# rland93/rrtplanner

Measured on AMD Instinct MI355X. Metric: RRT* nodes-expanded/s on 1024x1024 Perlin grid; achieved HBM GB/s, higher is better.
Workload: dtype int16x2 coordinates / u32 squared distances / f64 costs; 1 GPU; BASELINE.json configs[1]: RRT* 1024x1024 n=50000 r_rewire=64; queries_per_gpu=1, total_queries=1, n=50000, unfinished_queries=0, cus_per_query=65, pipelined=True, team_fallbacks=0, collective_library=librccl.so.1

## Files before the change

### include/rrt_hip.h

```cpp
#ifndef RRT_HIP_H
#define RRT_HIP_H

#include <stdint.h>

#ifdef __cplusplus
extern "C" {
#endif

#define RRT_OK 0
#define RRT_NEED_UNITBALL 1
#define RRT_E_ARG (-1)
#define RRT_E_GOAL_UNREACHABLE (-2)
#define RRT_E_HIP (-3)
#define RRT_E_NOGRID (-4)
#define RRT_E_UNSUPPORTED (-5)
#define RRT_E_COMM (-6)

#define RRT_ALG_STANDARD 0
#define RRT_ALG_STAR 1
#define RRT_ALG_INFORMED 2
#define RRT_ALG_DUBINS 3
#define RRT_ALG_DUBINS_STAR 4

#define RRT_FLAG_LOGS 1u
#define RRT_FLAG_SERIAL 2u
#define RRT_FLAG_NOTEAM 4u
#define RRT_FLAG_TEAM_FAULT 8u
#define RRT_FLAG_NOPIPE 16u
#define RRT_FLAG_REWIRE 32u
#define RRT_FLAG_DUBINS 64u
#define RRT_FLAG_NOPIPE1 32768u
#define RRT_FLAG_TEAM_MAX(g) ((uint32_t)(g) << 8)

typedef struct rrt_ctx rrt_ctx;
typedef struct rrt_batch rrt_batch;

typedef struct rrt_query {
    int32_t alg;
    int32_t n;
    int32_t xs[2];
    int32_t xg[2];
    int64_t r2_rewire;
    int64_t goal_d2;
    const int32_t *samples;
    double C[4];
    const int32_t *headings;
    double rho;
    int32_t nh;
    int32_t hs, hg;
    int32_t pad_;
    const uint32_t *samples_packed;
} rrt_query;

typedef struct rrt_result {
    int32_t *pts;
    double *vcost;
    int32_t *parent;
    int32_t *nearest_log;
    uint8_t *accept_log;
    double *cbest_log;
    int32_t *j_log;
    int32_t status;
    int32_t j;
// ... 76 lines not shown
```

### rrtplanner_amd/_ffi.py

```python
import ctypes as C
import weakref
import os

import numpy as np

_HERE = os.path.dirname(os.path.abspath(__file__))
LIB_PATH = os.environ.get("RRT_HIP_LIB", os.path.join(_HERE, "librrt_hip.so"))

RRT_OK = 0
RRT_NEED_UNITBALL = 1
RRT_E_ARG = -1
RRT_E_GOAL_UNREACHABLE = -2
RRT_E_HIP = -3
RRT_E_NOGRID = -4
RRT_E_UNSUPPORTED = -5
RRT_E_COMM = -6

ALG_STANDARD, ALG_STAR, ALG_INFORMED = 0, 1, 2
ALG_DUBINS, ALG_DUBINS_STAR = 3, 4
FLAG_LOGS = 1
FLAG_SERIAL = 2
FLAG_NOTEAM = 4
FLAG_TEAM_FAULT = 8
FLAG_NOPIPE = 16
FLAG_REWIRE = 32
FLAG_DUBINS = 64
FLAG_NOPIPE1 = 32768


def kernel_flags(logs=False, serial=False, team=None, team_fault=False, pipe=True, rewire=False, dubins=False, pipe1=True):
    f = (FLAG_LOGS if logs else 0) | (FLAG_SERIAL if serial else 0) | (FLAG_TEAM_FAULT if team_fault else 0) | (0 if pipe else FLAG_NOPIPE)
    f |= FLAG_REWIRE if rewire else 0
    f |= FLAG_DUBINS if dubins else 0
    f |= 0 if pipe1 else FLAG_NOPIPE1
    if team == 1:
        f |= FLAG_NOTEAM
    elif team is not None:
        if team not in (2, 3, 4, 8, 16, 32, 64):
            raise ValueError("team must be None, 1, 2, 3, 4, 8, 16, 32 or 64")
        f |= int(team) << 8
    return f

SYMBOLS = (
    "rrt_ctx_create", "rrt_ctx_destroy", "rrt_last_error_string", "rrt_set_grid", "rrt_noise_grids", "rrt_select_frame",
    "rrt_grid_generation", "rrt_ctx_sync",
    "rrt_comm_use_library", "rrt_comm_unique_id", "rrt_comm_init", "rrt_comm_destroy", "rrt_comm_allreduce_f64", "rrt_gather", "rrt_gather_fetch",
    "rrt_batch_create", "rrt_batch_destroy", "rrt_batch_set_query", "rrt_batch_set_unitball",
    "rrt_batch_rearm", "rrt_batch_launch", "rrt_batch_sync", "rrt_batch_team", "rrt_batch_team_info", "rrt_batch_pipelined", "rrt_batch_kernel_name", "rrt_batch_elapsed_ms",
    "rrt_batch_get_result", "rrt_batch_result_block", "rrt_batch_debug_cycles",
    "rrt_plan", "rrt_plan_resume", "rrt_plan_batch",
    "rrt_tree_create", "rrt_tree_destroy", "rrt_tree_reset", "rrt_tree_append", "rrt_tree_query",
    "rrt_prim_collisionfree", "rrt_prim_nearest_within", "rrt_prim_sqrt_u32", "rrt_prim_sqrt_u24", "rrt_prim_sqrt_f64",
)


class RRTError(RuntimeError):
    def __init__(self, code, msg):
        super().__init__(f"librrt_hip error {code}: {msg}")
        self.code = code


class Query(C.Structure):
    _fields_ = [
        ("alg", C.c_int32), ("n", C.c_int32),
        ("xs", C.c_int32 * 2), ("xg", C.c_int32 * 2),
        ("r2_rewire", C.c_int64), ("goal_d2", C.c_int64),
        ("samples", C.c_void_p),
# ... 199 lines not shown
                                              cells.ctypes.data, amps.ctypes.data, grads.ctypes.data, out.ctypes.data))
        self.shape = (W, H)
        return out

    def select_frame(self, k):
        _check(self._h, lib().rrt_select_frame(self._h, int(k)))

    def grid_generation(self):
        g = C.c_uint64(0)
        _check(self._h, lib().rrt_grid_generation(self._h, C.byref(g)))
        return g.value

    def sync(self):
        _check(self._h, lib().rrt_ctx_sync(self._h))

    def comm_init(self, rank, world, unique_id: bytes):
        if len(unique_id) != COMM_ID_BYTES:
            raise ValueError(f"unique id must have {COMM_ID_BYTES} bytes")
        buf = (C.c_uint8 * COMM_ID_BYTES).from_buffer_copy(unique_id)
        _check(self._h, lib().rrt_comm_init(self._h, int(rank), int(world), C.cast(buf, C.c_void_p)))
        self.rank, self.world = int(rank), int(world)

    def comm_destroy(self):
        _check(self._h, lib().rrt_comm_destroy(self._h))

    def allreduce(self, values, op="sum"):
        v = np.ascontiguousarray(values, dtype=np.float64).copy()
        _check(self._h, lib().rrt_comm_allreduce_f64(self._h, v.ctypes.data, v.size, {"sum": 0, "max": 1, "min": 2}[op]))
        return v

    def barrier(self):
        self.allreduce([0.0])

    def plan(self, query, n, logs=False, serial=False, team=None, team_fault=False, pipe=True, rewire=False, pipe1=True):
        res = ResultArrays(n, logs, headings=query.alg >= ALG_DUBINS)
        flags = kernel_flags(logs, serial, team, team_fault, pipe, rewire, pipe1=pipe1)
        rc = lib().rrt_plan(self._h, C.byref(query), flags, C.byref(res.c))
        _check(self._h, rc, ok=(RRT_OK, RRT_NEED_UNITBALL, RRT_E_GOAL_UNREACHABLE))
        return rc, res

    def plan_resume(self, unitball, res):
        ub = np.ascontiguousarray(unitball, dtype=np.float64)
        rc = lib().rrt_plan_resume(self._h, ub.ctypes.data, ub.shape[0], C.byref(res.c))
        _check(self._h, rc, ok=(RRT_OK, RRT_NEED_UNITBALL, RRT_E_GOAL_UNREACHABLE))
        return rc

    def plan_batch(self, queries, ns):
        Q = len(queries)
        qarr = (Query * Q)(*queries)
        res = [ResultArrays(int(n)) for n in ns]
        rarr = (Result * Q)(*[r.c for r in res])
        rc = lib().rrt_plan_batch(self._h, Q, qarr, rarr)
        _check(self._h, rc, ok=(RRT_OK, RRT_NEED_UNITBALL, RRT_E_GOAL_UNREACHABLE))
        for r, c in zip(res, rarr):
            r.c = c
        return rc, res

    def prim_collisionfree(self, ab):
        ab = np.ascontiguousarray(ab, dtype=np.int32).reshape(-1, 4)
        m = ab.shape[0]
        free = np.zeros(m, dtype=np.uint8)
        cells = np.zeros(m, dtype=np.int32)
        _check(self._h, lib().rrt_prim_collisionfree(self._h, ab.ctypes.data, m, free.ctypes.data, cells.ctypes.data))
        return free.astype(bool), cells

    def prim_nearest_within(self, pts, xq, r2):
        pts = np.ascontiguousarray(pts, dtype=np.int32).reshape(-1, 2)
        xq = np.ascontiguousarray(xq, dtype=np.int32).reshape(-1, 2)
        m = xq.shape[0]
# ... 33 lines not shown
        self._idx = np.zeros(self.capacity, dtype=np.int32)
        self._los = np.zeros(self.capacity + 1, dtype=np.uint8)

    def close(self):
        if self._h:
            lib().rrt_tree_destroy(self._h)
            self._h = C.c_void_p()

    def __del__(self):
        try:
            self.close()
        except Exception:
            pass

    def reset(self):
        _check(self.ctx.handle, lib().rrt_tree_reset(self._h))

    def append(self, x, y) -> int:
        j = C.c_int32(-1)
        _check(self.ctx.handle, lib().rrt_tree_append(self._h, int(x), int(y), C.byref(j)))
        return j.value

    def query(self, x, y, r2):
        nn, cnt = C.c_int32(-1), C.c_int32(0)
        _check(self.ctx.handle, lib().rrt_tree_query(self._h, int(x), int(y), int(r2), C.byref(nn), C.byref(cnt), self._idx.ctypes.data,
                                                     self._los.ctypes.data, self.capacity))
        m = cnt.value
        return nn.value, self._idx[:m].copy(), bool(self._los[0]), self._los[1:1 + m].astype(bool)


class Batch:

    def __init__(self, ctx: Context, Q: int, n_cap: int, logs: bool = False, serial: bool = False, team=None, team_fault: bool = False,
                 pipe: bool = True, rewire: bool = False, dubins: bool = False, pipe1: bool = True):
        self.ctx, self.Q, self.n_cap, self.logs, self.dubins = ctx, int(Q), int(n_cap), logs, dubins
        self._h = C.c_void_p()
        flags = kernel_flags(logs, serial, team, team_fault, pipe, rewire, dubins, pipe1)
        _check(ctx.handle, lib().rrt_batch_create(ctx.handle, self.Q, self.n_cap, flags, C.byref(self._h)))
        if not hasattr(ctx, "_batches"):
            ctx._batches = weakref.WeakSet()
        ctx._batches.add(self)
        self._n = [0] * self.Q

    def close(self):
        if self._h:
            lib().rrt_batch_destroy(self._h)
            self._h = C.c_void_p()

    def __del__(self):
        try:
            self.close()
        except Exception:
            pass

    def set_query(self, q, query):
        _check(self.ctx.handle, lib().rrt_batch_set_query(self._h, int(q), C.byref(query)))
        self._n[q] = query.n

    def set_unitball(self, q, unitball, ub_offset):
        ub = np.ascontiguousarray(unitball, dtype=np.float64)
        _check(self.ctx.handle, lib().rrt_batch_set_unitball(self._h, int(q), ub.ctypes.data, ub.shape[0], int(ub_offset)))

    def rearm(self):
        _check(self.ctx.handle, lib().rrt_batch_rearm(self._h))

    def launch(self):
        _check(self.ctx.handle, lib().rrt_batch_launch(self._h))

    def sync(self):
        _check(self.ctx.handle, lib().rrt_batch_sync(self._h))
# ... 57 lines not shown
```

### rrtplanner_amd/csrc/kernels_tu.hip

```cpp
#include <hip/hip_runtime.h>

#if RRT_TU == 1
#define RRT_BLOCK_DECL_ONLY
#define RRT_SERIAL_DECL_ONLY
#include "rrt_pipe.h"

#elif RRT_TU == 2
#include "rrt_dubins_block.h"
namespace rrtdev {
template __global__ void rrt_expand_kernel<false, true>(BatchView);
}

#elif RRT_TU == 3
#include "rrt_kernels.h"
namespace rrtdev {
template __global__ void rrt_expand_kernel<false, false>(BatchView);
template __global__ void rrt_expand_kernel<true, false>(BatchView);
}

#else
#define RRT_SERIAL_DECL_ONLY
#include "rrt_block.h"
namespace rrtdev {
#define K(G, BSM, PIPE, INF) template __global__ void rrt_expand_block_kernel<G, BSM, PIPE, INF>(BatchView);
#if RRT_TU == 10
K(64, 1, true, false)
#elif RRT_TU == 11
K(64, 1, true, true)
#elif RRT_TU == 12
K(32, 2, true, false) K(32, 2, true, true)
#elif RRT_TU == 13
K(16, 4, true, false) K(16, 4, true, true)
#elif RRT_TU == 14
K(8, 8, true, false) K(8, 8, true, true)
#elif RRT_TU == 15
K(4, 16, true, false) K(4, 16, true, true)
#elif RRT_TU == 16
K(3, 16, true, false) K(3, 16, true, true)
#elif RRT_TU == 17
K(2, 16, true, false) K(2, 16, true, true) K(2, 32, true, false)
#elif RRT_TU == 18
K(64, 1, false, false) K(64, 1, false, true) K(32, 2, false, false) K(32, 2, false, true)
#elif RRT_TU == 19
K(16, 4, false, false) K(16, 4, false, true) K(8, 8, false, false) K(8, 8, false, true)
#elif RRT_TU == 20
K(4, 16, false, false) K(4, 16, false, true) K(2, 16, false, false) K(2, 16, false, true)
#elif RRT_TU == 21
K(1, 16, false, false) K(1, 16, false, true)
#else
#error "RRT_TU: unknown translation unit"
#endif
#undef K
}
#endif
```

### rrtplanner_amd/csrc/rrt_block.h

```cpp
#pragma once

#include "rrt_kernels.h"

namespace rrtdev {

constexpr int BS = 16;

constexpr int TEAM_MAX = 64;
#ifndef RRT_PIPE_LAG
#define RRT_PIPE_LAG 2
#endif
#ifndef RRT_PIPE_LAG_SMALL
#define RRT_PIPE_LAG_SMALL 1
#endif
#ifndef RRT_PIPE_LAG_INF
#define RRT_PIPE_LAG_INF 2
#endif
#ifndef RRT_NPMAX
#define RRT_NPMAX 2
#endif
constexpr int NPMAX = RRT_NPMAX;
#ifndef RRT_PL_MAX
#define RRT_PL_MAX 12
#endif
// ... 759 lines not shown
#ifdef RRT_STAMPS
    if (lane == 0 && !PIPE) {
        D->wcyc[wave] = wcyc_acc;
        D->wcyc[16 + wave] = wcyc_los;
    }
    if (PIPE && t == 0 && g <= 1)
#pragma unroll
        for (int k = 0; k < 16; ++k) D->wcyc[16 * g + k] = dbg[k];
#endif
}

template <int G, int BSM, bool PIPE, bool INF>
__global__ __launch_bounds__(TPB) void rrt_expand_block_kernel(BatchView bv)
#ifdef RRT_BLOCK_DECL_ONLY
    ;
#else
{
    __shared__ BlockLds<G, BSM, PIPE, INF> L;
    if constexpr (PIPE) {
#if defined(RRT_ONLY_ROLE) && RRT_ONLY_ROLE == 1
        rrt_block_body<G, BSM, PIPE, INF, ROLE_COMMIT>(bv, L);
#elif defined(RRT_ONLY_ROLE) && RRT_ONLY_ROLE == 2
        rrt_block_body<G, BSM, PIPE, INF, ROLE_WORK>(bv, L);
#else
        if ((int)blockIdx.x < bv.team_qpad) rrt_block_body<G, BSM, PIPE, INF, ROLE_COMMIT>(bv, L);
        else rrt_block_body<G, BSM, PIPE, INF, ROLE_WORK>(bv, L);
#endif
    } else {
        rrt_block_body<G, BSM, PIPE, INF, ROLE_ALL>(bv, L);
    }
}
#endif

}
```

### rrtplanner_amd/csrc/rrt_block_nearset.inc

```

    constexpr bool GQ = PIPE && ROLE == ROLE_WORK && BSM < 16;
    constexpr uint32_t OQCAP = (uint32_t)(SB * BREC_WORDS * 8 / 16 / (BSM < 16 ? BSM : 1));
    constexpr bool GLIST = false;
    constexpr bool LDSLIST = BSM >= 16 || GLIST;
    constexpr uint32_t LCAP = BSM >= 16 ? (uint32_t)BLOCK_LIST_CAP : (uint32_t)(SB * BREC_WORDS * 8 / 16 / NWAVE);
    const uint32_t clist_cap = (uint32_t)(bv.spill_stride / (2 * NWAVE * (G + (PIPE ? 1 : 0))));
    u32x4 *const clist_base = reinterpret_cast<u32x4 *>(spill) + (size_t)(g * NWAVE) * (size_t)clist_cap;
    u32x4 *const clist = clist_base + (size_t)wave * (size_t)clist_cap;
    RRT_LDS u32x4 *const clist_l =
        GLIST ? (RRT_LDS u32x4 *)&brec[PIPE ? 1 : 0][0] + (size_t)wave * LCAP
              : (RRT_LDS u32x4 *)(smem + (size_t)lds_chunks * CHUNK * sizeof(uint32_t) + (size_t)MAX_CELLS * sizeof(uint32_t)) + (size_t)wave * LCAP;
    auto lget = [&](uint32_t p) -> u32x4 {
        if (LDSLIST && p < LCAP) return clist_l[p];
        return clist[p];
    };
    auto lput = [&](uint32_t p, u32x4 e) {
        if (LDSLIST && p < LCAP) clist_l[p] = e;
        else clist[p] = e;
    };
    auto lput_y = [&](uint32_t p, uint32_t y) {
        if (LDSLIST && p < LCAP) clist_l[p].y = y;
        else clist[p].y = y;
    };
    RRT_LDS u32x4 *const clist_l0 = clist_l - (size_t)wave * LCAP;
// ... 46 lines not shown
        uint32_t ld2 = NONE, lidx = NONE;
        nlist = 0;
        float T = boundf;
        uint32_t Thi = hi_of((double)boundf);
        auto eval_record = [&](const u32x4 rc, bool &dirty) {
            const uint32_t d2 = dist2(rc.x, X);
            const bool hit = d2 < r2h && (!check_j0 || rc.y < (uint32_t)j0);
            hits += hit ? 1u : 0u;
            if (hit && (d2 < ld2 || (d2 == ld2 && rc.y < lidx))) {
                ld2 = d2;
                lidx = rc.y;
                lxy = rc.x;
                lvlo = rc.z;
                lvhi = rc.w;
            }
            if (!star) return;
            const bool park = hit && rc.w <= boundhi;
            const unsigned long long pm = __ballot(park);
            if (pm == 0) return;
            if (park) {
                const uint32_t pos = nlist + (uint32_t)__builtin_popcountll(pm & ((1ull << lane) - 1ull));
                if (pos < clist_cap) lput(pos, u32x4{rc.y, rc.x, rc.z, rc.w});
            }
            nlist += (uint32_t)__builtin_popcountll(pm);
            const bool pre = park && rc.w <= Thi;
            if (__ballot(pre) == 0) return;
            const double V = __longlong_as_double((long long)(((unsigned long long)rc.w << 32) | rc.z));
            const bool maybe = pre && ((float)V + __builtin_amdgcn_sqrtf((float)d2) < T);
            if (__ballot(maybe) == 0) return;
            if (maybe) {
                const double cn = V + sqrt_u24(d2);
                const bool in = cn < bound && !key_lt(cn, rc.y, lbc, lbi);
                if (in) {
                    if (key_lt(cn, rc.y, tt.c1, tt.i1)) {
                        fx2 = fx1;
                        fx1 = rc.x;
                    } else if (key_lt(cn, rc.y, tt.c2, tt.i2)) {
                        fx2 = rc.x;
                    }
                    tt.fold(cn, rc.y);
                }
                const float cu = in ? screen_of(cn) : FINF;
                const float lo = __builtin_fminf(m1, cu), hi = __builtin_fmaxf(m1, cu);
                m1 = lo;
                m2 = __builtin_fminf(m2, hi);
            }
            dirty = true;
        };
        auto tighten = [&]() {
            const float w1 = wave_min_f32_nonneg(m1);
            const float w2 = wave_min_f32_nonneg(m1 == w1 ? m2 : m1);
            T = w2 < boundf ? w2 : boundf;
            Thi = hi_of((double)T);
        };
        for (int cbase = 0; cbase < ncr; cbase += 64) {
            uint32_t tcnt = 0, toff = 0;
            if (cbase + lane < ncr) {
                const int ci = cbase + lane, ccx = cx0 + ci / ny, ccy = cy0 + ci % ny, cell = ccx * ncy + ccy;
#ifndef RRT_NO_CELL_CULL
                const int xl = ccx << cshift, xh = xl + (1 << cshift) - 1, yl = ccy << cshift, yh = yl + (1 << cshift) - 1;
                const int ddx = x < xl ? xl - x : (x > xh ? x - xh : 0), ddy = y < yl ? yl - y : (y > yh ? y - yh : 0);
                tcnt = (uint32_t)(ddx * ddx + ddy * ddy) < r2h ? cellcnt[cell] : 0u;
#else
                tcnt = cellcnt[cell];
#endif
                toff = (uint32_t)cell * (uint32_t)ccap;
            }
            uint32_t incl = tcnt;
            incl += (uint32_t)__builtin_amdgcn_update_dpp(0, (int)incl, 0x111, 0xf, 0xf, false);
            incl += (uint32_t)__builtin_amdgcn_update_dpp(0, (int)incl, 0x112, 0xf, 0xf, false);
            incl += (uint32_t)__builtin_amdgcn_update_dpp(0, (int)incl, 0x114, 0xf, 0xf, false);
            incl += (uint32_t)__builtin_amdgcn_update_dpp(0, (int)incl, 0x118, 0xf, 0xf, false);
// ... 262 lines not shown
```

### rrtplanner_amd/csrc/rrt_engine.hip

```cpp
#include <hip/hip_runtime.h>
#include <rccl/rccl.h>
#include <dlfcn.h>

#include <chrono>
#include <cmath>
#include <cstdarg>
#include <cstdio>
#include <cstdlib>
#include <cstring>
#include <mutex>
#include <string>
#include <tuple>
#include <vector>

#define RRT_BLOCK_DECL_ONLY
#define RRT_SERIAL_DECL_ONLY
#include "rrt_hip.h"
#include "rrt_kernels.h"
#include "rrt_block.h"
#include "rrt_kernel_decls.h"
#include "rrt_prims.h"

using namespace rrtdev;

static thread_local std::string g_last_error;

constexpr int RRT_GRID_FAST = 2048;
constexpr int RRT_GRID_MAX = 32767;

struct PinnedDescs {
    QDesc *p = nullptr;
    size_t n = 0;
    hipError_t alloc(size_t count) {
        release();
        hipError_t e = hipHostMalloc(reinterpret_cast<void **>(&p), count * sizeof(QDesc), hipHostMallocDefault);
        if (e != hipSuccess) {
            p = nullptr;
            return e;
        }
        n = count;
        for (size_t k = 0; k < n; ++k) p[k] = QDesc{};
        return hipSuccess;
    }
    void release() {
        if (p) (void)hipHostFree(p);
        p = nullptr;
        n = 0;
    }
    QDesc *data() { return p; }
    QDesc *begin() { return p; }
    QDesc *end() { return p + n; }
    QDesc &operator[](size_t k) { return p[k]; }
};

struct rrt_ctx {
    int device = 0;
    hipStream_t stream = nullptr;
    uint8_t *og = nullptr;
    uint8_t *og_buf = nullptr;
    size_t og_buf_bytes = 0;
    int32_t nframes = 1;
    int32_t W = 0, H = 0;
    std::string err;
    rrt_batch *single = nullptr;
    uint32_t single_flags = 0;
    int max_lds = 0;
    int num_cu = 0;
    uint64_t grid_gen = 0;
    ncclComm_t comm = nullptr;
    int32_t comm_rank = 0, comm_world = 1;
    unsigned char *gather_buf = nullptr;
    size_t gather_bytes = 0;
    const rrt_batch *gather_owner = nullptr;
    double *d_red = nullptr;
};

struct rrt_batch {
    rrt_ctx *ctx = nullptr;
    int32_t Q = 0, n_cap = 0, node_stride = 0, bitmap_words = 0, lds_chunks = 1, spill_stride = 0;
    int32_t gridW = 0, gridH = 0;
    uint32_t flags = 0;
    bool use_block = false;
    bool dub_block = false;
    int32_t blk_lds_chunks = 1;
    int32_t blk_lds_chunks16 = 1;
    int32_t team = 1;
    bool pipe_team = false;
    bool pipe = false;
    int32_t last_team = 0;
    bool last_inf = false;
    bool last_pipe1 = false;
    bool last_wide = false;
    int32_t team_fallbacks = 0;
    int32_t team_qpad = 0;
    int32_t team_want = TEAM_MAX;
    int32_t claimed_cus = 0;
    int32_t shrunk = 0;
    unsigned char *d_team = nullptr;
    QDesc *d_desc = nullptr;
    PinnedDescs h_desc;
    size_t serial_lds_static = 0;
    uint32_t *d_samples = nullptr, *d_nodes = nullptr, *d_bitmap = nullptr;
    double *d_vcost = nullptr, *d_unitball = nullptr, *d_cbest_log = nullptr;
    int32_t *d_parent = nullptr, *d_nearest_log = nullptr, *d_j_log = nullptr;
    uint8_t *d_accept_log = nullptr;
    uint2 *d_spill = nullptr;
    int32_t *d_kids = nullptr;
    uint32_t *d_frontier = nullptr;
    int32_t *d_vsoln = nullptr;
    uint8_t *d_heading = nullptr;
    uint8_t *d_shead = nullptr;
    double *d_dubpath = nullptr;
    std::vector<uint8_t> stage8;
    uint4 *d_cellrec = nullptr;
    uint32_t *d_cellcnt = nullptr;
    int64_t rec_stride = 0;
    unsigned char *d_slab = nullptr;
    size_t slab_bytes = 0;
    hipEvent_t ev0 = nullptr, ev1 = nullptr;
    bool timed = false;
    float ms_before = 0.f;
    bool one_cu_once = false;
    std::vector<uint32_t> stage;
};

static const void *block_kernel_of(int team, bool pipe, bool inf);
static size_t block_kernel_static_lds(int team);

static hipError_t raise_dynamic_lds(int device, const void *kern, int bytes) {
    static std::mutex mu;
    static std::vector<std::tuple<int, const void *, int>> have;
    std::lock_guard<std::mutex> lock(mu);
    for (auto &t : have)
        if (std::get<0>(t) == device && std::get<1>(t) == kern) {
            if (std::get<2>(t) >= bytes) return hipSuccess;
            const hipError_t e = hipFuncSetAttribute(kern, hipFuncAttributeMaxDynamicSharedMemorySize, bytes);
            if (e == hipSuccess) std::get<2>(t) = bytes;
            return e;
        }
    const hipError_t e = hipFuncSetAttribute(kern, hipFuncAttributeMaxDynamicSharedMemorySize, bytes);
    if (e == hipSuccess) have.emplace_back(device, kern, bytes);
    return e;
}

static int fail(rrt_ctx *ctx, int code, const char *fmt, ...) {
    char buf[512];
    va_list ap;
    va_start(ap, fmt);
    vsnprintf(buf, sizeof buf, fmt, ap);
    va_end(ap);
    g_last_error = buf;
    if (ctx) ctx->err = buf;
// ... 34 lines not shown
        return e;
    }
};

extern "C" const char *rrt_last_error_string(rrt_ctx *ctx) { return ctx ? ctx->err.c_str() : g_last_error.c_str(); }

extern "C" int rrt_ctx_create(int32_t device_id, rrt_ctx **out) {
    if (!out) return fail(nullptr, RRT_E_ARG, "rrt_ctx_create: out is NULL");
    int ndev = 0;
    HIPCHK(nullptr, hipGetDeviceCount(&ndev));
    if (device_id < 0 || device_id >= ndev)
        return fail(nullptr, RRT_E_ARG, "rrt_ctx_create: device %d of %d", device_id, ndev);
    HIPCHK(nullptr, hipSetDevice(device_id));
    rrt_ctx *c = new rrt_ctx();
    c->device = device_id;
    hipError_t e = hipStreamCreateWithFlags(&c->stream, hipStreamNonBlocking);
    if (e == hipSuccess) e = hipDeviceGetAttribute(&c->max_lds, hipDeviceAttributeMaxSharedMemoryPerBlock, device_id);
    if (e == hipSuccess) e = hipDeviceGetAttribute(&c->num_cu, hipDeviceAttributeMultiprocessorCount, device_id);
    if (e != hipSuccess) {
        if (c->stream) (void)hipStreamDestroy(c->stream);
        delete c;
        return fail(nullptr, RRT_E_HIP, "rrt_ctx_create: %s", hipGetErrorString(e));
    }
    *out = c;
    return RRT_OK;
}

extern "C" int rrt_ctx_destroy(rrt_ctx *ctx) {
    if (!ctx) return RRT_OK;
    (void)hipSetDevice(ctx->device);
    if (ctx->single) rrt_batch_destroy(ctx->single);
    (void)rrt_comm_destroy(ctx);
    if (ctx->og_buf) (void)hipFree(ctx->og_buf);
    if (ctx->stream) (void)hipStreamDestroy(ctx->stream);
    delete ctx;
    return RRT_OK;
}

extern "C" int rrt_set_grid(rrt_ctx *ctx, const uint8_t *og_nonzero, int32_t W, int32_t H) {
    if (!ctx || !og_nonzero || W < 1 || H < 1) return fail(ctx, RRT_E_ARG, "rrt_set_grid: bad argument");
    if (W > RRT_GRID_MAX || H > RRT_GRID_MAX)
        return fail(ctx, RRT_E_UNSUPPORTED, "rrt_set_grid: %dx%d exceeds %d cells per axis (16-bit packed coordinates)", W, H, RRT_GRID_MAX);
    HIPCHK(ctx, hipSetDevice(ctx->device));
    HIPCHK(ctx, hipStreamSynchronize(ctx->stream));
    if (ctx->og_buf && ctx->og_buf_bytes != (size_t)W * H) {
        ctx->grid_gen += 1;
        ctx->og = nullptr;
        HIPCHK(ctx, hipFree(ctx->og_buf));
        ctx->og_buf = nullptr;
    }
    if (!ctx->og_buf) {
        HIPCHK(ctx, hipMalloc(&ctx->og_buf, (size_t)W * H));
        ctx->og_buf_bytes = (size_t)W * H;
    }
    ctx->og = ctx->og_buf;
    ctx->nframes = 1;
    ctx->grid_gen += 1;
    HIPCHK(ctx, hipMemcpyAsync(ctx->og, og_nonzero, (size_t)W * H, hipMemcpyHostToDevice, ctx->stream));
    HIPCHK(ctx, hipStreamSynchronize(ctx->stream));
    ctx->W = W;
    ctx->H = H;
    return RRT_OK;
}

namespace {
__device__ __forceinline__ double fade5(double t) { return t * t * t * (t * (t * 6.0 - 15.0) + 10.0); }
// ... 161 lines not shown

namespace {
std::mutex g_cu_mutex;
std::vector<int> g_cu_claimed;
int cu_claim(int device, int num_cu, int want_cus, int min_cus) {
    std::lock_guard<std::mutex> lock(g_cu_mutex);
    if ((int)g_cu_claimed.size() <= device) g_cu_claimed.resize((size_t)device + 1, 0);
    const int free_cus = num_cu - g_cu_claimed[(size_t)device];
    if (want_cus <= free_cus || want_cus <= min_cus) {
        g_cu_claimed[(size_t)device] += want_cus;
        return -1;
    }
    return free_cus < 0 ? 0 : free_cus;
}
void cu_release(int device, int cus) {
    if (cus <= 0) return;
    std::lock_guard<std::mutex> lock(g_cu_mutex);
    if ((int)g_cu_claimed.size() > device) g_cu_claimed[(size_t)device] -= cus;
}
}

extern "C" int rrt_batch_destroy(rrt_batch *b) {
    if (!b) return RRT_OK;
    (void)hipSetDevice(b->ctx->device);
    (void)hipStreamSynchronize(b->ctx->stream);
    void *ptrs[] = {b->d_desc,  b->d_samples,   b->d_slab,        b->d_bitmap, b->d_unitball,  b->d_cellrec,
                    b->d_spill, b->d_cbest_log, b->d_nearest_log, b->d_j_log,  b->d_accept_log, b->d_cellcnt,
                    b->d_team,  b->d_kids,      b->d_frontier,    b->d_vsoln,  b->d_heading,   b->d_shead,
                    b->d_dubpath};
    for (void *p : ptrs)
        if (p) (void)hipFree(p);
    if (b->ev0) (void)hipEventDestroy(b->ev0);
    if (b->ev1) (void)hipEventDestroy(b->ev1);
    cu_release(b->ctx->device, b->claimed_cus);
    b->claimed_cus = 0;
    if (b->ctx->single == b) b->ctx->single = nullptr;
    if (b->ctx->gather_owner == b) b->ctx->gather_owner = nullptr;
    b->h_desc.release();
    delete b;
    return RRT_OK;
}

struct TeamShape {
    int team = 1, qpad = 0;
    bool pipe = false;
    int cus() const { return team > 1 ? qpad * (team + (pipe ? 1 : 0)) : 0; }
};
static TeamShape pick_team(int Q, int want, bool allow_pipe, int cus);
static bool two_cus_run_the_pipeline(const rrt_batch *b);
static TeamShape pick_team(int Q, int want, bool allow_pipe, int cus) {
    TeamShape t;
    t.qpad = (Q + 7) & ~7;
    auto stride_of = [&](int g) {
        const int step = g <= 16 ? 8 : (g == 32 ? 4 : 2);
        int stride = ((Q + step - 1) / step) * step;
        if (g == 32 && stride % 8 == 0) stride += 4;
        if (g == 64 && stride % 4 == 0) stride += 2;
        return stride;
    };
    for (int g : {2, 4, 8, 16, 32, 64})
        if (g <= want && stride_of(g) * g <= cus) {
            t.team = g;
            t.qpad = stride_of(g);
        }
    int pipe_g = 0;
    if (allow_pipe)
// ... 288 lines not shown
    if constexpr (!INF) {
        if (pipe && wide && team == 2) return rrt_expand_block_kernel<2, 32, true, false>;
    }
    if (pipe) {
        switch (team) {
            case 64: return rrt_expand_block_kernel<64, 1, true, INF>;
            case 32: return rrt_expand_block_kernel<32, 2, true, INF>;
            case 16: return rrt_expand_block_kernel<16, 4, true, INF>;
            case 8: return rrt_expand_block_kernel<8, 8, true, INF>;
            case 4: return rrt_expand_block_kernel<4, 16, true, INF>;
            case 3: return rrt_expand_block_kernel<3, 16, true, INF>;
            default: return rrt_expand_block_kernel<2, 16, true, INF>;
        }
    }
    switch (team) {
        case 64: return rrt_expand_block_kernel<64, 1, false, INF>;
        case 32: return rrt_expand_block_kernel<32, 2, false, INF>;
        case 16: return rrt_expand_block_kernel<16, 4, false, INF>;
        case 8: return rrt_expand_block_kernel<8, 8, false, INF>;
        case 4: return rrt_expand_block_kernel<4, 16, false, INF>;
        case 2: return rrt_expand_block_kernel<2, 16, false, INF>;
        default: return rrt_expand_block_kernel<1, 16, false, INF>;
    }
}

static block_kernel_fn block_kernel_fn_of(int team, bool pipe, bool inf, bool wide = false) {
    return inf ? block_kernel_fn_inf<true>(team, pipe, wide) : block_kernel_fn_inf<false>(team, pipe, wide);
}

static const void *block_kernel_of(int team, bool pipe, bool inf, bool wide = false) {
    return reinterpret_cast<const void *>(block_kernel_fn_of(team, pipe, inf, wide));
}

static size_t block_kernel_static_lds(int team) {
    hipFuncAttributes a{};
    size_t worst = 0;
    for (int g : {1, 2, 3, 4, 8, 16, 32, 64})
        for (bool pipe : {false, true})
            for (bool inf : {false, true}) {
                if (g > team || (pipe && g < 2)) continue;
                if (!pipe && g == 3) continue;
                for (bool wide : {false, true}) {
                    if (wide && !(pipe && g == 2)) continue;
                    if (hipFuncGetAttributes(&a, block_kernel_of(g, pipe, inf, wide)) != hipSuccess) return 16384;
                    worst = a.sharedSizeBytes > worst ? a.sharedSizeBytes : worst;
                }
            }
    return (worst + 255) & ~(size_t)255;
}

static size_t expand_lds_bytes(int lds_chunks) {
    return (size_t)lds_chunks * CHUNK * sizeof(uint32_t);
}

static bool two_cus_run_the_pipeline(const rrt_batch *b) {
    return b->use_block && b->team == 2 && !b->pipe_team && b->team_want >= TEAM_MAX && !(b->flags & (RRT_FLAG_NOPIPE | RRT_FLAG_NOPIPE1));
}

extern "C" int rrt_batch_launch(rrt_batch *b) {
    if (!b) return fail(nullptr, RRT_E_ARG, "rrt_batch_launch: NULL");
    rrt_ctx *ctx = b->ctx;
    if (!ctx->og) return fail(ctx, RRT_E_NOGRID, "rrt_batch_launch: no grid");
    if (b->gridW != ctx->W || b->gridH != ctx->H) return fail(ctx, RRT_E_ARG, "rrt_batch_launch: grid changed shape");
    HIPCHK(ctx, hipSetDevice(ctx->device));
    if (!b->one_cu_once) b->ms_before = 0.f;
    BatchView v = make_view(b);
// ... 27 lines not shown
            if (ts.team != team) b->shrunk += 1;
            team = ts.team;
            pipe_shape = ts.pipe;
            v.team_qpad = ts.qpad;
            b->claimed_cus = team > 1 ? ts.cus() : 0;
        }
        if (team <= 1) {
            team = 1;
            b->claimed_cus = b->Q < ctx->num_cu ? b->Q : ctx->num_cu;
            (void)cu_claim(ctx->device, ctx->num_cu, b->claimed_cus, b->claimed_cus);
        }
        const bool lists = team <= 4;
        v.lds_chunks = lists ? b->blk_lds_chunks16 : b->blk_lds_chunks;
        const size_t blk_lds_bytes = (size_t)MAX_CELLS * sizeof(uint32_t) + (lists ? BLOCK_LIST_LDS_BYTES : 0) + (size_t)v.lds_chunks * CHUNK * sizeof(uint32_t);
        bool pipe = team > 1 && pipe_shape;
#ifdef RRT_STAMPS
        if (const char *e = getenv("RRT_PIPE")) pipe = pipe && atoi(e) != 0;
#endif
        b->pipe = pipe;
        bool inf = false;
        for (const QDesc &d : b->h_desc)
            if (d.status == ST_RUNNING && d.alg == 2) inf = true;
#ifndef RRT_NO_WIDE
        bool wide = pipe && !inf && team == 2;
        for (const QDesc &d : b->h_desc)
            if (d.status == ST_RUNNING && d.alg != RRT_ALG_STANDARD && d.r2_rewire < 257u) wide = false;
#else
        const bool wide = false;
#endif
        b->last_wide = wide;
        b->last_team = team;
        b->last_inf = inf;
        b->last_pipe1 = false;
        if (team == 1 && !inf && !continuation && !(b->flags & RRT_FLAG_NOPIPE1)) {
            b->last_pipe1 = true;
            hipLaunchKernelGGL(rrt_init_kernel<0>, ig, dim3(256), 0, ctx->stream, v);
            HIPCHK(ctx, hipEventRecord(b->ev0, ctx->stream));
            hipLaunchKernelGGL(rrt_pipe_kernel, dim3((unsigned)b->Q), dim3(TPB), 0, ctx->stream, v);
            HIPCHK(ctx, hipEventRecord(b->ev1, ctx->stream));
            HIPCHK(ctx, hipGetLastError());
            b->timed = true;
            return RRT_OK;
        }
        HIPCHK(ctx, raise_dynamic_lds(ctx->device, block_kernel_of(team, pipe, inf, wide), (int)blk_lds_bytes));
        hipLaunchKernelGGL(rrt_init_kernel<0>, ig, dim3(256), 0, ctx->stream, v);
        if (team > 1) HIPCHK(ctx, hipMemsetAsync(b->d_team, 0, (size_t)b->Q * TEAM_BYTES, ctx->stream));
        HIPCHK(ctx, hipEventRecord(b->ev0, ctx->stream));
        const dim3 tg(team > 1 ? (unsigned)(v.team_qpad * (team + (pipe ? 1 : 0))) : (unsigned)b->Q);
        hipLaunchKernelGGL(block_kernel_fn_of(team, pipe, inf, wide), tg, dim3(TPB), blk_lds_bytes, ctx->stream, v);
        HIPCHK(ctx, hipEventRecord(b->ev1, ctx->stream));
        HIPCHK(ctx, hipGetLastError());
        b->timed = true;
        return RRT_OK;
    }
    cu_release(ctx->device, b->claimed_cus);
    b->claimed_cus = b->Q < ctx->num_cu ? b->Q : ctx->num_cu;
    (void)cu_claim(ctx->device, ctx->num_cu, b->claimed_cus, b->claimed_cus);
    if (b->dub_block) {
        hipLaunchKernelGGL(rrt_init_kernel<0>, ig, dim3(256), 0, ctx->stream, v);
        HIPCHK(ctx, hipEventRecord(b->ev0, ctx->stream));
        hipLaunchKernelGGL(rrt_dubins_block_kernel, dim3((unsigned)b->Q), dim3(TPB), 0, ctx->stream, v);
        HIPCHK(ctx, hipEventRecord(b->ev1, ctx->stream));
        HIPCHK(ctx, hipGetLastError());
        b->timed = true;
        return RRT_OK;
    }
    const size_t lds = expand_lds_bytes(b->lds_chunks);
    typedef void (*serial_kernel_fn)(BatchView);
    const serial_kernel_fn kern = (b->flags & RRT_FLAG_DUBINS)  ? static_cast<serial_kernel_fn>(rrt_expand_kernel<false, true>)
                                  : (b->flags & RRT_FLAG_REWIRE) ? static_cast<serial_kernel_fn>(rrt_expand_kernel<true, false>)
                                                                 : static_cast<serial_kernel_fn>(rrt_expand_kernel<false, false>);
    if (b->serial_lds_static == 0) {
        hipFuncAttributes fa{};
        HIPCHK(ctx, hipFuncGetAttributes(&fa, reinterpret_cast<const void *>(kern)));
        b->serial_lds_static = fa.sharedSizeBytes + 1;
    }
    const size_t lds_static = b->serial_lds_static - 1;
    if ((int)(lds + lds_static) > ctx->max_lds) return fail(ctx, RRT_E_HIP, "LDS request %zu exceeds %d", lds + lds_static, ctx->max_lds);
    HIPCHK(ctx, raise_dynamic_lds(ctx->device, reinterpret_cast<const void *>(kern), (int)lds));
    hipLaunchKernelGGL(rrt_init_kernel<0>, ig, dim3(256), 0, ctx->stream, v);
    HIPCHK(ctx, hipEventRecord(b->ev0, ctx->stream));
    hipLaunchKernelGGL(kern, dim3((unsigned)b->Q), dim3(TPB), lds, ctx->stream, v);
// ... 64 lines not shown
    }
    return RRT_OK;
}

extern "C" int rrt_batch_team(rrt_batch *b, int32_t *cus_per_query, int32_t *fallbacks) {
    if (!b || !cus_per_query) return fail(nullptr, RRT_E_ARG, "rrt_batch_team: NULL");
    *cus_per_query = b->use_block ? b->team : 1;
    if (fallbacks) *fallbacks = b->team_fallbacks;
    return RRT_OK;
}

extern "C" int rrt_batch_team_info(rrt_batch *b, int32_t out[4]) {
    if (!b || !out) return fail(nullptr, RRT_E_ARG, "rrt_batch_team_info: NULL");
    out[0] = b->use_block ? b->team : 1;
    out[1] = b->use_block ? (b->last_team > 0 ? b->last_team : b->team) : 1;
    out[2] = b->team_fallbacks;
    out[3] = b->shrunk;
    return RRT_OK;
}

extern "C" int rrt_batch_pipelined(rrt_batch *b, int32_t *pipelined) {
    if (!b || !pipelined) return fail(nullptr, RRT_E_ARG, "rrt_batch_pipelined: NULL");
    *pipelined = (b->use_block && b->team > 1 && b->pipe) ? 1 : 0;
    return RRT_OK;
}

extern "C" int rrt_batch_kernel_name(rrt_batch *b, char *buf, int32_t len) {
    if (!b || !buf || len < 1) return fail(nullptr, RRT_E_ARG, "rrt_batch_kernel_name: bad argument");
    char tmp[160];
    if (b->use_block) {
        const int team = b->last_team > 0 ? b->last_team : b->team;
        const int bsm = b->last_wide ? 32 : (team <= 4 ? 16 : 64 / team);
        if (b->last_pipe1) snprintf(tmp, sizeof tmp, "rrt_pipe_kernel");
        else snprintf(tmp, sizeof tmp, "rrt_expand_block_kernel<%d, %d, %s, %s>", team, bsm, (team > 1 && b->pipe) ? "true" : "false", b->last_inf ? "true" : "false");
    } else if (b->dub_block) {
        snprintf(tmp, sizeof tmp, "rrt_dubins_block_kernel");
    } else {
        snprintf(tmp, sizeof tmp, "rrt_expand_kernel<%s, %s>", (b->flags & RRT_FLAG_REWIRE) ? "true" : "false", (b->flags & RRT_FLAG_DUBINS) ? "true" : "false");
    }
    snprintf(buf, (size_t)len, "%s", tmp);
    return RRT_OK;
}

extern "C" int rrt_batch_elapsed_ms(rrt_batch *b, float *ms) {
    if (!b || !ms) return fail(nullptr, RRT_E_ARG, "rrt_batch_elapsed_ms: NULL");
    if (!b->timed) return fail(b->ctx, RRT_E_ARG, "rrt_batch_elapsed_ms: nothing launched");
    HIPCHK(b->ctx, hipEventElapsedTime(ms, b->ev0, b->ev1));
    *ms += b->ms_before;
    return RRT_OK;
}

extern "C" int rrt_batch_get_result(rrt_batch *b, int32_t q, rrt_result *out) {
    if (!b || !out) return fail(nullptr, RRT_E_ARG, "rrt_batch_get_result: NULL");
    rrt_ctx *ctx = b->ctx;
    if (q < 0 || q >= b->Q) return fail(ctx, RRT_E_ARG, "rrt_batch_get_result: q=%d of %d", q, b->Q);
    HIPCHK(ctx, hipSetDevice(ctx->device));
    const QDesc &d = b->h_desc[(size_t)q];
    if (d.status == ST_RUNNING || d.status == ST_IDLE)
        return fail(ctx, RRT_E_ARG, "rrt_batch_get_result: query %d has not run (launch + sync first)", q);
    out->status = d.status;
    out->j = d.j;
    out->vgoal = d.vgoal;
    out->found = d.found;
    out->i_switch = d.i_switch;
    out->rows = d.found ? d.n + 1 : d.n;
    out->sum_j = (int64_t)d.sum_j;
// ... 564 lines not shown
```

Baseline: 6.000 million nodes/s.

## Split pipelined team kernel into separate commit and work kernels on two streams

For pipelined teams of 8 or more, the single fused block kernel is replaced by a commit kernel (512 threads, one block per query) launched on a second stream and a work kernel on the main stream, joined by events. Each role can then be compiled with its own launch bounds and register budget instead of sharing one body. The near-set update is also rewritten from nested branches into branchless selects. The two kernels rely on co-residency for their inter-block handshake, which creates deadlock or scheduling risk if they are not both resident.

```diff
diff --git a/include/rrt_hip.h b/include/rrt_hip.h
--- a/include/rrt_hip.h
+++ b/include/rrt_hip.h
@@ -29,6 +29,7 @@
 #define RRT_FLAG_NOPIPE 16u
 #define RRT_FLAG_REWIRE 32u
 #define RRT_FLAG_DUBINS 64u
+#define RRT_FLAG_ONEBODY 128u
 #define RRT_FLAG_NOPIPE1 32768u
 #define RRT_FLAG_TEAM_MAX(g) ((uint32_t)(g) << 8)
 
diff --git a/rrtplanner_amd/_ffi.py b/rrtplanner_amd/_ffi.py
--- a/rrtplanner_amd/_ffi.py
+++ b/rrtplanner_amd/_ffi.py
@@ -25,14 +25,16 @@
 FLAG_NOPIPE = 16
 FLAG_REWIRE = 32
 FLAG_DUBINS = 64
+FLAG_ONEBODY = 128
 FLAG_NOPIPE1 = 32768
 
 
-def kernel_flags(logs=False, serial=False, team=None, team_fault=False, pipe=True, rewire=False, dubins=False, pipe1=True):
+def kernel_flags(logs=False, serial=False, team=None, team_fault=False, pipe=True, rewire=False, dubins=False, pipe1=True, onebody=False):
     f = (FLAG_LOGS if logs else 0) | (FLAG_SERIAL if serial else 0) | (FLAG_TEAM_FAULT if team_fault else 0) | (0 if pipe else FLAG_NOPIPE)
     f |= FLAG_REWIRE if rewire else 0
     f |= FLAG_DUBINS if dubins else 0
     f |= 0 if pipe1 else FLAG_NOPIPE1
+    f |= FLAG_ONEBODY if onebody else 0
     if team == 1:
         f |= FLAG_NOTEAM
     elif team is not None:
@@ -298,9 +300,9 @@
     def barrier(self):
         self.allreduce([0.0])
 
-    def plan(self, query, n, logs=False, serial=False, team=None, team_fault=False, pipe=True, rewire=False, pipe1=True):
+    def plan(self, query, n, logs=False, serial=False, team=None, team_fault=False, pipe=True, rewire=False, pipe1=True, onebody=False):
         res = ResultArrays(n, logs, headings=query.alg >= ALG_DUBINS)
-        flags = kernel_flags(logs, serial, team, team_fault, pipe, rewire, pipe1=pipe1)
+        flags = kernel_flags(logs, serial, team, team_fault, pipe, rewire, pipe1=pipe1, onebody=onebody)
         rc = lib().rrt_plan(self._h, C.byref(query), flags, C.byref(res.c))
         _check(self._h, rc, ok=(RRT_OK, RRT_NEED_UNITBALL, RRT_E_GOAL_UNREACHABLE))
         return rc, res
@@ -400,10 +402,10 @@
 class Batch:
 
     def __init__(self, ctx: Context, Q: int, n_cap: int, logs: bool = False, serial: bool = False, team=None, team_fault: bool = False,
-                 pipe: bool = True, rewire: bool = False, dubins: bool = False, pipe1: bool = True):
+                 pipe: bool = True, rewire: bool = False, dubins: bool = False, pipe1: bool = True, onebody: bool = False):
         self.ctx, self.Q, self.n_cap, self.logs, self.dubins = ctx, int(Q), int(n_cap), logs, dubins
         self._h = C.c_void_p()
-        flags = kernel_flags(logs, serial, team, team_fault, pipe, rewire, dubins, pipe1)
+        flags = kernel_flags(logs, serial, team, team_fault, pipe, rewire, dubins, pipe1, onebody)
         _check(ctx.handle, lib().rrt_batch_create(ctx.handle, self.Q, self.n_cap, flags, C.byref(self._h)))
         if not hasattr(ctx, "_batches"):
             ctx._batches = weakref.WeakSet()
diff --git a/rrtplanner_amd/csrc/kernels_tu.hip b/rrtplanner_amd/csrc/kernels_tu.hip
--- a/rrtplanner_amd/csrc/kernels_tu.hip
+++ b/rrtplanner_amd/csrc/kernels_tu.hip
@@ -23,6 +23,9 @@
 #include "rrt_block.h"
 namespace rrtdev {
 #define K(G, BSM, PIPE, INF) template __global__ void rrt_expand_block_kernel<G, BSM, PIPE, INF>(BatchView);
+#define S(G, BSM, INF)                                                        \
+    template __global__ void rrt_block_commit_kernel<G, BSM, INF>(BatchView); \
+    template __global__ void rrt_block_work_kernel<G, BSM, INF>(BatchView);
 #if RRT_TU == 10
 K(64, 1, true, false)
 #elif RRT_TU == 11
@@ -47,9 +50,16 @@
 K(4, 16, false, false) K(4, 16, false, true) K(2, 16, false, false) K(2, 16, false, true)
 #elif RRT_TU == 21
 K(1, 16, false, false) K(1, 16, false, true)
+#elif RRT_TU == 22
+S(64, 1, false)
+#elif RRT_TU == 23
+S(32, 2, false)
+#elif RRT_TU == 24
+S(16, 4, false) S(8, 8, false)
 #else
 #error "RRT_TU: unknown translation unit"
 #endif
 #undef K
+#undef S
 }
 #endif
diff --git a/rrtplanner_amd/csrc/rrt_block.h b/rrtplanner_amd/csrc/rrt_block.h
--- a/rrtplanner_amd/csrc/rrt_block.h
+++ b/rrtplanner_amd/csrc/rrt_block.h
@@ -815,4 +815,26 @@
 }
 #endif
 
-}
+template <int G, int BSM, bool INF>
+__global__ __launch_bounds__(512) void rrt_block_commit_kernel(BatchView bv)
+#ifdef RRT_BLOCK_DECL_ONLY
+    ;
+#else
+{
+    __shared__ BlockLds<G, BSM, true, INF> L;
+    rrt_block_body<G, BSM, true, INF, ROLE_COMMIT, 8>(bv, L);
+}
+#endif
+
+template <int G, int BSM, bool INF>
+__global__ __launch_bounds__(TPB) void rrt_block_work_kernel(BatchView bv)
+#ifdef RRT_BLOCK_DECL_ONLY
+    ;
+#else
+{
+    __shared__ BlockLds<G, BSM, true, INF> L;
+    rrt_block_body<G, BSM, true, INF, ROLE_WORK>(bv, L);
+}
+#endif
+
+}
diff --git a/rrtplanner_amd/csrc/rrt_block_nearset.inc b/rrtplanner_amd/csrc/rrt_block_nearset.inc
--- a/rrtplanner_amd/csrc/rrt_block_nearset.inc
+++ b/rrtplanner_amd/csrc/rrt_block_nearset.inc
@@ -102,12 +102,10 @@
                 const double cn = V + sqrt_u24(d2);
                 const bool in = cn < bound && !key_lt(cn, rc.y, lbc, lbi);
                 if (in) {
-                    if (key_lt(cn, rc.y, tt.c1, tt.i1)) {
-                        fx2 = fx1;
-                        fx1 = rc.x;
-                    } else if (key_lt(cn, rc.y, tt.c2, tt.i2)) {
-                        fx2 = rc.x;
-                    }
+                    const bool b1 = key_lt(cn, rc.y, tt.c1, tt.i1);
+                    const bool b2 = key_lt(cn, rc.y, tt.c2, tt.i2);
+                    fx2 = b1 ? fx1 : (b2 ? rc.x : fx2);
+                    fx1 = b1 ? rc.x : fx1;
                     tt.fold(cn, rc.y);
                 }
                 const float cu = in ? screen_of(cn) : FINF;
diff --git a/rrtplanner_amd/csrc/rrt_engine.hip b/rrtplanner_amd/csrc/rrt_engine.hip
--- a/rrtplanner_amd/csrc/rrt_engine.hip
+++ b/rrtplanner_amd/csrc/rrt_engine.hip
@@ -56,6 +56,7 @@
 struct rrt_ctx {
     int device = 0;
     hipStream_t stream = nullptr;
+    hipStream_t stream2 = nullptr;
     uint8_t *og = nullptr;
     uint8_t *og_buf = nullptr;
     size_t og_buf_bytes = 0;
@@ -91,6 +92,7 @@
     bool last_inf = false;
     bool last_pipe1 = false;
     bool last_wide = false;
+    bool last_split = false;
     int32_t team_fallbacks = 0;
     int32_t team_qpad = 0;
     int32_t team_want = TEAM_MAX;
@@ -118,6 +120,7 @@
     unsigned char *d_slab = nullptr;
     size_t slab_bytes = 0;
     hipEvent_t ev0 = nullptr, ev1 = nullptr;
+    hipEvent_t ev_fork = nullptr, ev_join = nullptr;
     bool timed = false;
     float ms_before = 0.f;
     bool one_cu_once = false;
@@ -218,6 +221,7 @@
     if (ctx->single) rrt_batch_destroy(ctx->single);
     (void)rrt_comm_destroy(ctx);
     if (ctx->og_buf) (void)hipFree(ctx->og_buf);
+    if (ctx->stream2) (void)hipStreamDestroy(ctx->stream2);
     if (ctx->stream) (void)hipStreamDestroy(ctx->stream);
     delete ctx;
     return RRT_OK;
@@ -445,6 +449,8 @@
         if (p) (void)hipFree(p);
     if (b->ev0) (void)hipEventDestroy(b->ev0);
     if (b->ev1) (void)hipEventDestroy(b->ev1);
+    if (b->ev_fork) (void)hipEventDestroy(b->ev_fork);
+    if (b->ev_join) (void)hipEventDestroy(b->ev_join);
     cu_release(b->ctx->device, b->claimed_cus);
     b->claimed_cus = 0;
     if (b->ctx->single == b) b->ctx->single = nullptr;
@@ -799,6 +805,19 @@
     return reinterpret_cast<const void *>(block_kernel_fn_of(team, pipe, inf, wide));
 }
 
+static bool split_team(int team, bool pipe, bool inf, bool wide, uint32_t flags) {
+    return pipe && !inf && !wide && team >= 8 && !(flags & RRT_FLAG_ONEBODY);
+}
+
+static void split_kernels_of(int team, block_kernel_fn &commit, block_kernel_fn &work) {
+    switch (team) {
+        case 64: commit = rrt_block_commit_kernel<64, 1, false>, work = rrt_block_work_kernel<64, 1, false>; break;
+        case 32: commit = rrt_block_commit_kernel<32, 2, false>, work = rrt_block_work_kernel<32, 2, false>; break;
+        case 16: commit = rrt_block_commit_kernel<16, 4, false>, work = rrt_block_work_kernel<16, 4, false>; break;
+        default: commit = rrt_block_commit_kernel<8, 8, false>, work = rrt_block_work_kernel<8, 8, false>; break;
+    }
+}
+
 static size_t block_kernel_static_lds(int team) {
     hipFuncAttributes a{};
     size_t worst = 0;
@@ -892,6 +911,7 @@
         b->last_team = team;
         b->last_inf = inf;
         b->last_pipe1 = false;
+        b->last_split = false;
         if (team == 1 && !inf && !continuation && !(b->flags & RRT_FLAG_NOPIPE1)) {
             b->last_pipe1 = true;
             hipLaunchKernelGGL(rrt_init_kernel<0>, ig, dim3(256), 0, ctx->stream, v);
@@ -902,12 +922,35 @@
             b->timed = true;
             return RRT_OK;
         }
-        HIPCHK(ctx, raise_dynamic_lds(ctx->device, block_kernel_of(team, pipe, inf, wide), (int)blk_lds_bytes));
+        const bool split = split_team(team, pipe, inf, wide, b->flags);
+        block_kernel_fn kcommit = nullptr, kwork = nullptr;
+        if (split) {
+            split_kernels_of(team, kcommit, kwork);
+            if (!ctx->stream2) HIPCHK(ctx, hipStreamCreateWithFlags(&ctx->stream2, hipStreamNonBlocking));
+            if (!b->ev_fork) HIPCHK(ctx, hipEventCreateWithFlags(&b->ev_fork, hipEventDisableTiming));
+            if (!b->ev_join) HIPCHK(ctx, hipEventCreateWithFlags(&b->ev_join, hipEventDisableTiming));
+            HIPCHK(ctx, raise_dynamic_lds(ctx->device, reinterpret_cast<const void *>(kcommit), (int)blk_lds_bytes));
+            HIPCHK(ctx, raise_dynamic_lds(ctx->device, reinterpret_cast<const void *>(kwork), (int)blk_lds_bytes));
+        } else {
+            HIPCHK(ctx, raise_dynamic_lds(ctx->device, block_kernel_of(team, pipe, inf, wide), (int)blk_lds_bytes));
+        }
         hipLaunchKernelGGL(rrt_init_kernel<0>, ig, dim3(256), 0, ctx->stream, v);
         if (team > 1) HIPCHK(ctx, hipMemsetAsync(b->d_team, 0, (size_t)b->Q * TEAM_BYTES, ctx->stream));
         HIPCHK(ctx, hipEventRecord(b->ev0, ctx->stream));
-        const dim3 tg(team > 1 ? (unsigned)(v.team_qpad * (team + (pipe ? 1 : 0))) : (unsigned)b->Q);
-        hipLaunchKernelGGL(block_kernel_fn_of(team, pipe, inf, wide), tg, dim3(TPB), blk_lds_bytes, ctx->stream, v);
+        if (split) {
+            HIPCHK(ctx, hipEventRecord(b->ev_fork, ctx->stream));
+            HIPCHK(ctx, hipStreamWaitEvent(ctx->stream2, b->ev_fork, 0));
+            hipLaunchKernelGGL(kcommit, dim3((unsigned)v.team_qpad), dim3(512), blk_lds_bytes, ctx->stream2, v);
+            BatchView vw = v;
+            vw.member0 = 1;
+            hipLaunchKernelGGL(kwork, dim3((unsigned)(v.team_qpad * team)), dim3(TPB), blk_lds_bytes, ctx->stream, vw);
+            HIPCHK(ctx, hipEventRecord(b->ev_join, ctx->stream2));
+            HIPCHK(ctx, hipStreamWaitEvent(ctx->stream, b->ev_join, 0));
+            b->last_split = true;
+        } else {
+            const dim3 tg(team > 1 ? (unsigned)(v.team_qpad * (team + (pipe ? 1 : 0))) : (unsigned)b->Q);
+            hipLaunchKernelGGL(block_kernel_fn_of(team, pipe, inf, wide), tg, dim3(TPB), blk_lds_bytes, ctx->stream, v);
+        }
         HIPCHK(ctx, hipEventRecord(b->ev1, ctx->stream));
         HIPCHK(ctx, hipGetLastError());
         b->timed = true;
@@ -1038,6 +1081,9 @@
         const int team = b->last_team > 0 ? b->last_team : b->team;
         const int bsm = b->last_wide ? 32 : (team <= 4 ? 16 : 64 / team);
         if (b->last_pipe1) snprintf(tmp, sizeof tmp, "rrt_pipe_kernel");
+        else if (b->last_split)
+            snprintf(tmp, sizeof tmp, "rrt_expand_block_kernel<%d, %d, true, false> as rrt_block_commit_kernel + rrt_block_work_kernel<%d, %d, false>", team,
+                     bsm, team, bsm);
         else snprintf(tmp, sizeof tmp, "rrt_expand_block_kernel<%d, %d, %s, %s>", team, bsm, (team > 1 && b->pipe) ? "true" : "false", b->last_inf ? "true" : "false");
     } else if (b->dub_block) {
         snprintf(tmp, sizeof tmp, "rrt_dubins_block_kernel");
```

Result: faster. 6.275 million nodes/s (median of 6 runs) (+4.6%).
